# 2noise/ChatTTS

Hardware: AMD Instinct MI355X
Metric: audio seconds/sec (RTF), batch=64 per GPU (higher is better)
Workload: dtype f32x3

## Files before the change

### chattts_amd/_lib.py

```python
from __future__ import annotations

import ctypes as C
import os

import numpy as np

import torch

HERE = os.path.dirname(os.path.abspath(__file__))
LIB_PATH = os.environ.get("CTTS_LIB") or os.path.join(HERE, "csrc", "libchattts_amd.so")

F32, BF16 = 0, 1
P = C.c_void_p
PP = C.POINTER(C.c_void_p)


class GptWeights(C.Structure):
    _fields_ = [
        ("n_layers", C.c_int32), ("weight_dtype", C.c_int32), ("kv_dtype", C.c_int32), ("max_pos", C.c_int32),
        ("wqkv", PP), ("wo", PP), ("wgu", PP), ("wd", PP), ("ln1", PP), ("ln2", PP),
        ("norm", P), ("emb_code", P), ("heads", P), ("rope_cos", P), ("rope_sin", P),
        ("rms_eps", C.c_float),
        ("emb_text", P), ("head_text", P), ("n_text", C.c_int32),
        ("wqkv_pk", PP), ("wo_pk", PP), ("wgu_pk", PP), ("wd_pk", PP),
        ("heads_pk", P), ("head_text_pk", P),
        ("wo_hd", PP),
        ("wqkv_x3", PP), ("wo_x3", PP), ("wgu_x3", PP), ("wd_x3", PP),
    ]


class GenState(C.Structure):
    _fields_ = [
        ("B", C.c_int32), ("T", C.c_int32), ("max_new", C.c_int32),
        ("ids_buf", P), ("len", P), ("kv_start", P), ("finish", P), ("end_idx", P), ("hiddens", P),
        ("kcache", P), ("vcache", P), ("q", P), ("nq", C.c_int32),
        ("temperature", P), ("pow_table", P),
        ("top_p_thr", C.c_float), ("use_top_p", C.c_int32), ("top_k", C.c_int32), ("use_top_k", C.c_int32),
        ("min_new", C.c_int32), ("eos", C.c_int32), ("row_offset", C.c_int32),
        ("stop_at", P), ("workspace", P), ("workspace_bytes", C.c_size_t), ("row_map", P), ("n_active", P),
        ("cap", C.c_int32), ("hid_cap", C.c_int32), ("kv_batch", C.c_int32), ("q_batch", C.c_int32), ("prompt_len", P),
        ("infer_text", C.c_int32), ("teacher_ids", P), ("sampled_ids", P), ("order", P),
        ("rng_device", C.c_int32), ("rng_per_step", C.c_int32), ("rng_seed", P), ("rng_nonce", P),
# ... 106 lines not shown
    "ctts_dvae_encode_workspace_bytes": (SZ, [I32]),
    "ctts_dvae_decode_workspace_bytes": (SZ, [I32, I32]),
    "ctts_dvae_encode": (C.c_int, [P, P, I32, P, P, SZ, P]),
    "ctts_dvae_decode_codes": (C.c_int, [P, P, P, I32, I32, P, SZ, P]),
    "ctts_k_gemm": (C.c_int, [I32, P, P, P, I32, I32, I32, I32, I32, I32, I32, P, F, P, I32, P, P, I32, I32, I32, I32, I32, P]),
    "ctts_k_gemm_x3p": (C.c_int, [P, P, I32, I32, I32, I32, P, P, P, P, P, P]),
    "ctts_k_gemm_h1p": (C.c_int, [P, P, I32, I32, I32, I32, P, P, P, P, P, P]),
    "ctts_stream_create_cu_mask": (C.c_int, [I32, I32, I32, I32, P]),
    "ctts_stream_destroy": (C.c_int, [P]),
    "ctts_k_mlp_fused": (C.c_int, [P, P, P, I32, I32, P, P, P, P, I32, P]),
    "ctts_k_gemm_fast": (C.c_int, [P, I32, P, I32, I32, I32, P, F, I32, P, I32, P, I32, P, P]),
    "ctts_k_qkv_rope": (C.c_int, [P, P, I32, P, F, P, P, P, I32, P, P, I32, P, P, I32, P]),
    "ctts_k_gemm_dec": (C.c_int, [P, P, I32, I32, I32, P, P, F, I32, P, I32, P, I32, P, I32, P]),
    "ctts_k_gemm_dec32x": (C.c_int, [P, C.c_int64, P, C.c_int64, I32, I32, I32, P, P, I32, F, I32, P, I32, P, I32, P, C.c_int64, I32, P, I32, P, P, P]),
    "ctts_k_gemm_pre_x3": (C.c_int, [P, I32, P, P, I32, I32, I32, I32, I32, P, P, P, I32, P]),
    "ctts_k_dec32_last_variant": (C.c_char_p, []),
    "ctts_k_gemm_dec32": (C.c_int, [P, P, I32, I32, I32, P, P, I32, P, F, I32, P, I32, P, I32, P, I32, I32, I32, P]),
    "ctts_k_rows_prep": (C.c_int, [P, P, P, I32, P]),
    "ctts_k_rope_append": (C.c_int, [P, P, P, I32, I32, P, P, I32, P, P, I32, P]),
    "ctts_k_attention": (C.c_int, [P, P, P, I32, I32, P, I32, P, P, I32, P]),
    "ctts_k_attention_prefill": (C.c_int, [P, P, P, I32, P, I32, I32, P, I32, P]),
    "ctts_k_attention_dec": (C.c_int, [P, P, P, I32, P, P, P, I32, P, P, I32, P]),
    "ctts_k_attention_dec2": (C.c_int, [P, P, P, I32, I32, P, P, P, I32, I32, P]),
    "ctts_k_attention_cfg": (C.c_int, [I32, I32, I32]),
    "ctts_k_attention_heads_per_wg": (C.c_int, [I32]),
    "ctts_rccl_unique_id": (C.c_int, [P]),
    "ctts_rccl_comm_create": (C.c_int, [P, I32, P, I32]),
    "ctts_rccl_comm_destroy": (None, [P]),
    "ctts_broadcast_weights": (C.c_int, [P, P, I32, P, I32, P]),
    "ctts_k_attention_oproj": (C.c_int, [P, P, P, I32, P, P, P, I32, P, P, P, P, P, P]),
# ... 48 lines not shown
```

### chattts_amd/csrc/capi.hip

```cpp
#include <hip/hip_runtime.h>
#include <dlfcn.h>
#include <stdarg.h>
#include <stdio.h>
#include <stdlib.h>
#include <string.h>
#include <algorithm>
#include <map>
#include <vector>

#include "../../include/chattts_amd.h"
#include "kernels.hpp"

static thread_local char g_err[512] = "";
int ctts_fail(const char* fmt, ...) {
  va_list ap;
  va_start(ap, fmt);
  vsnprintf(g_err, sizeof(g_err), fmt, ap);
  va_end(ap);
  return -1;
}
#define fail ctts_fail
#define CK(expr)                                                                                   \
  do {                                                                                             \
    hipError_t _e = (expr);                                                                        \
// ... 11 lines not shown
  std::vector<const void*> wqkv_pk, wo_pk, wgu_pk, wd_pk;
  std::vector<const void*> wo_hd;
  std::vector<const void*> wqkv_x3, wo_x3, wgu_x3, wd_x3;
  bool dec_x3 = false;
  bool qkv_att = false;
  bool att_oproj = false;
  bool dec_packed = false;
  bool dec_packed32 = false;
  bool heads_packed = false;
  int pf_mask = 0;
  int temporal_layers = 0;
  bool pre32_packed = true;
  bool embed_fold = false;
  bool pre_compact = true;
  bool pre_x3 = true;
  bool fnorm_fuse = true;
  std::vector<const float*> ln1, ln2;
  hipGraph_t graph = nullptr;
  hipGraphExec_t exec = nullptr;
  hipGraph_t graph_multi = nullptr;
  hipGraphExec_t exec_multi = nullptr;
  struct RowsGraph { hipGraph_t graph = nullptr, gm = nullptr; hipGraphExec_t exec = nullptr, exec_multi = nullptr; };
  std::map<int, RowsGraph> rows_graphs;
  int multi_steps = 1;
  int prof_tag = -1;
  int prof_max = 0;
  bool skip_finished = true;
  int n_cu = 0;
  int prof_stride = 1;
  int prof_seen = 0;
// ... 92 lines not shown
    g->dec_x3 = true;
  }
  if (w->wo_hd && g->dec_packed) {
    g->wo_hd.assign(w->wo_hd, w->wo_hd + L);
    const char* e = getenv("CTTS_ATT_OPROJ");
    g->att_oproj = e && atoi(e) == 1;
  }
  { const char* e = getenv("CTTS_SKIP_FINISHED"); if (e && atoi(e) == 0) g->skip_finished = false; }
  { const char* e = getenv("CTTS_FNORM_FUSE"); if (e && atoi(e) == 0) g->fnorm_fuse = false; }
  { const char* e = getenv("CTTS_W_TEMPORAL_LAYERS"); if (e) g->temporal_layers = atoi(e); }
  { const char* e = getenv("CTTS_PF"); if (e) g->pf_mask = atoi(e); }
  { const char* e = getenv("CTTS_QKV_ATT"); g->qkv_att = e && atoi(e) == 1; }
  { const char* e = getenv("CTTS_PRE32_PACKED"); if (e && atoi(e) == 0) g->pre32_packed = false; }
  { const char* e = getenv("CTTS_PRE_X3"); if (e && atoi(e) == 0) g->pre_x3 = false; }
  { const char* e = getenv("CTTS_PRE_COMPACT"); if (e && atoi(e) == 0) g->pre_compact = false; }
  { const char* e = getenv("CTTS_EMBED_FOLD"); if (e) g->embed_fold = atoi(e) != 0; }
  {
    int dev = 0, cus = 0;
    const char* e = getenv("CTTS_ATT_SPLIT");
    if (e && atoi(e) == 1 && hipGetDevice(&dev) == hipSuccess &&
        hipDeviceGetAttribute(&cus, hipDeviceAttributeMultiprocessorCount, dev) == hipSuccess && cus > 0 && cus <= ATT_CUS_MAX)
      g->n_cu = cus;
  }
  *out = g;
  return 0;
}

extern "C" void ctts_gpt_graph_destroy(ctts_gpt* g) {
  if (!g) return;
  if (g->exec) { (void)hipGraphExecDestroy(g->exec); g->exec = nullptr; }
// ... 254 lines not shown
    d.epi = D32_EPI_QKV_ROPE; d.C = ws.qkv; d.ldc = 3 * HID; d.desc = ws.desc; d.cos_t = g->w.rope_cos; d.sin_t = g->w.rope_sin;
    d.kc = (float*)kc; d.vc = (float*)vc; d.cmax = cmax;
    CK(launch_gemm_pre32(d, ws.rstd, st));
    CK(launch_attention(ws.qkv, kc, vc, kt, cmax, ws.aop32, 3, rm, M, st));
    d.Ap = ws.aop32; d.Wp = (const float*)g->wo_pk[l]; d.N = HID; d.norm_w = nullptr; d.epi = EPI_RES; d.C = ws.x; d.ldc = HID;
    d.res = ws.x; d.ldr = HID; d.Cp = ws.xp32; d.kch_out = HID / 16;
    CK(launch_gemm_pre32(d, nullptr, st));
    CK(launch_rows_rstd32(ws.x, HID, M, g->w.rms_eps, ws.rstd, st));
    d.Ap = ws.xp32; d.Wp = (const float*)g->wgu_pk[l]; d.N = INTER; d.norm_w = g->ln2[l]; d.epi = EPI_SILU_MUL; d.C = nullptr;
    d.res = nullptr; d.Cp = ws.actp32; d.kch_out = INTER / 16;
    CK(launch_gemm_pre32(d, ws.rstd, st));
    d.Ap = ws.actp32; d.Wp = (const float*)g->wd_pk[l]; d.N = HID; d.K = INTER; d.norm_w = nullptr; d.epi = EPI_RES;
    d.C = ws.x; d.ldc = HID; d.res = ws.x; d.ldr = HID; d.Cp = ws.xp32; d.kch_out = HID / 16;
    CK(launch_gemm_pre32(d, nullptr, st));
  }
  for (int l = 0; !fast && !packed32 && !pre32 && !x3 && l < g->w.n_layers; ++l) {
    void* kc = (char*)s->kcache + kv_layer * l;
    void* vc = (char*)s->vcache + kv_layer * l;
    GemmArgs a;
    memset(&a, 0, sizeof(a));
    a.taps = 1;
    a.n_active = nact;
    a.A = ws.x; a.lda = HID; a.W = g->wqkv[l]; a.C = ws.qkv; a.ldc = 3 * HID; a.M = M; a.N = 3 * HID; a.K = HID; a.wt = wt;
    a.epi = EPI_STORE; a.norm_w = g->ln1[l]; a.eps = g->w.rms_eps;
    if (pre_x3) { CK(launch_rows_rstd32(ws.x, HID, M, g->w.rms_eps, ws.rstd, st)); CK(launch_gemm_pre_x3(a, ws.rstd, st)); }
    else { Prof p(g, 1, st, prof_ok); CK(launch_gemm_skinny(a, st)); }
    { Prof p(g, 2, st, prof_ok); CK(launch_rope_append(ws.qkv, kc, vc, kt, cmax, g->w.rope_cos, g->w.rope_sin, rm, M, st)); }
    { Prof p(g, 3, st, prof_ok); CK(launch_attention(ws.qkv, kc, vc, kt, cmax, ws.ao, 0, rm, M, st)); }
    a.A = ws.ao; a.lda = HID; a.W = g->wo[l]; a.C = ws.x; a.ldc = HID; a.N = HID; a.K = HID; a.epi = EPI_RES; a.norm_w = nullptr;
    a.res = ws.x; a.ldr = HID;
    if (pre_x3) CK(launch_gemm_pre_x3(a, nullptr, st));
// ... 837 lines not shown
}
extern "C" int ctts_k_final_norm(const float* x, int32_t q_per_b, const float* w, float eps, float* hfin, float* hiddens,
                                 int32_t max_new, const int32_t* len, int32_t T, int32_t B, void* stream) {
  CK(launch_final_norm(x, q_per_b, w, eps, hfin, hiddens, max_new, len, T, B, nullptr, nullptr, nullptr, (hipStream_t)stream));
  return 0;
}
extern "C" int ctts_k_gemm_pre_x3(const float* A, int32_t lda, const float* W, float* C, int32_t ldc, int32_t M, int32_t N, int32_t K, int32_t epi,
                                  const float* norm_w, const float* rstd, const float* res, int32_t ldr, void* stream) {
  GemmArgs a;
  memset(&a, 0, sizeof(a));
  a.taps = 1; a.A = A; a.lda = lda; a.W = W; a.C = C; a.ldc = ldc; a.M = M; a.N = N; a.K = K; a.wt = WT_F32; a.epi = epi;
  a.norm_w = norm_w; a.res = res; a.ldr = ldr;
  CK(launch_gemm_pre_x3(a, rstd, (hipStream_t)stream));
  return 0;
}
extern "C" int ctts_k_sample(const ctts_gen_state* s, const float* logits, void* stream) {
  if (!s || !logits) return fail("ctts_k_sample: bad arguments");
  CK(launch_sample(make_sample_args(s, logits), (hipStream_t)stream));
  return 0;
}
extern "C" int ctts_k_sample_text(const ctts_gen_state* s, const float* logits, int32_t n_text, void* stream) {
  if (!s || !logits || n_text <= 0 || n_text > NTEXT_MAX) return fail("ctts_k_sample_text: bad arguments");
  CK(launch_sample_text(make_sample_args(s, logits), n_text, (hipStream_t)stream));
  return 0;
}
extern "C" int ctts_k_device_guard_probe(void* stream, int32_t* before, int32_t* stream_dev, int32_t* inside, int32_t* switched) {
  if (!before || !stream_dev || !inside || !switched) return fail("ctts_k_device_guard_probe: null argument");
  int b = -1, in = -1;
  CK(hipGetDevice(&b));
  *stream_dev = -1;
// ... 252 lines not shown
```

### chattts_amd/csrc/gpt.hip

```cpp
#include <stdlib.h>

#include "common.hpp"
#include "kernels.hpp"
#include "decode_dev.hpp"

#ifndef CTTS_QF_DELAY
#define CTTS_QF_DELAY 8
#endif
#ifndef CTTS_QF_PRE
#define CTTS_QF_PRE 1
#endif
#define HID 768
#define NHEAD 12
#define HDIM 64
#define NVQ 4
#define NAUDIO 626

__device__ __forceinline__ void row_to_b_slot(const GptRowMap& rm, int m, int& b, int& slot) {
  if (rm.q_per_b == 1) { b = rm.row_map ? rm.row_map[m] : m; slot = rm.len[b] - 1; }
  else { b = m / rm.q_per_b; slot = rm.slot0 + m - b * rm.q_per_b; if (rm.row_map) b = rm.row_map[b]; }
}
__device__ __forceinline__ bool row_absent(const int32_t* n_active, int m) { return n_active != nullptr && m >= *n_active; }

__device__ __forceinline__ void emit_row(float4 s, int t, float* __restrict__ x_row, uint16_t* __restrict__ xb_row,
// ... 245 lines not shown
template <> __device__ __forceinline__ size_t pko_off<x3p_t>(int m, int c) { return pk_off(m, c, HID / 32); }
template <typename OT> __device__ __forceinline__ void store_out(OT* p, float v);
template <> __device__ __forceinline__ void store_out<x3p_t>(x3p_t* p, float v) { p->v = f32_to_bf16(v); }
template <typename OT> __device__ __forceinline__ void store_pko(OT* out, int m, int c, float v, size_t);
template <> __device__ __forceinline__ void store_pko<x3p_t>(x3p_t* out, int m, int c, float v, size_t plane) {
  uint16_t* p = reinterpret_cast<uint16_t*>(out) + pk_off(m, c, HID / 32);
  uint16_t h, l;
  x3_split(v, h, l);
  p[0] = h;
  p[plane] = l;
}
template <> __device__ __forceinline__ void store_out<float>(float* p, float v) { *p = v; }
template <> __device__ __forceinline__ void store_out<bf16_t>(bf16_t* p, float v) { *p = f32_to_bf16(v); }
template <> __device__ __forceinline__ void store_pko<float>(float* out, int m, int c, float v, size_t) { out[pko_off<float>(m, c)] = v; }
template <> __device__ __forceinline__ void store_pko<bf16_t>(bf16_t* out, int m, int c, float v, size_t) { out[pko_off<bf16_t>(m, c)] = f32_to_bf16(v); }

#ifndef CTTS_ATT_DPP
#define CTTS_ATT_DPP 1
#endif
template <int CTRL>
__device__ __forceinline__ float dpp_f(float v) {
  return __int_as_float(__builtin_amdgcn_update_dpp(__float_as_int(v), __float_as_int(v), CTRL, 0xf, 0xf, false));
}
template <int LPK>
__device__ __forceinline__ float group_sum(float d) {
#if CTTS_ATT_DPP
  d += dpp_f<0xB1>(d);
  d += dpp_f<0x4E>(d);
  d += dpp_f<0x141>(d);
  if (LPK == 16) d += dpp_f<0x140>(d);
// ... 314 lines not shown
    const u128* wo = reinterpret_cast<const u128*>(rm.wo_h) + (size_t)h * 8 * HID + tid;
#pragma unroll
    for (int jc = 0; jc < 3; ++jc)
#pragma unroll
      for (int g8 = 0; g8 < 8; ++g8) wv[jc][g8] = load16(wo + (size_t)g8 * HID + 256 * jc);
    __builtin_amdgcn_sched_barrier(0);
  }
  lrun = groups_sum<LPK>(lrun, lane);
#pragma unroll
  for (int e = 0; e < DPL; ++e) acc[e] = groups_sum<LPK>(acc[e], lane);
  if (NW == 1) {
    if (kg == 0) {
      const float inv = 1.0f / lrun;
      OT* op = PKO ? out + pko_off<OT>(m, h * HDIM + dl * DPL) : out + (size_t)m * HID + h * HDIM + dl * DPL;
#pragma unroll
      for (int e = 0; e < DPL; ++e) store_out<OT>(op + e, acc[e] * inv);
    }
    return;
  }
  if (kg == 0) {
    if (dl == 0) { sm_m[wave] = mrun; sm_l[wave] = lrun; }
#pragma unroll
    for (int e = 0; e < DPL; ++e) sm_acc[wave][dl * DPL + e] = acc[e];
  }
  __syncthreads();
  if (tid < HDIM) {
    float M = -INFINITY;
#pragma unroll
    for (int w = 0; w < NW; ++w) M = fmaxf(M, sm_m[w]);
    float L = 0.f, o = 0.f;
#pragma unroll
// ... 516 lines not shown
      CTTS_LAUNCH_SMEM((attention_k<bf16_t, 16, bf16_t, true>), grid, dim3(1024), att_lds, st, qkv, (const bf16_t*)kcache, (const bf16_t*)vcache, cmax, (bf16_t*)out, rm);
    else if (att_nbuf == 3)
      CTTS_LAUNCH_SMEM((attention_k<bf16_t, 4, bf16_t, true, false, false, 3>), grid, dim3(256), att_lds, st, qkv, (const bf16_t*)kcache, (const bf16_t*)vcache, cmax, (bf16_t*)out, rm);
    else
      CTTS_LAUNCH_SMEM((attention_k<bf16_t, 4, bf16_t, true>), grid, dim3(256), att_lds, st, qkv, (const bf16_t*)kcache, (const bf16_t*)vcache, cmax, (bf16_t*)out, rm);
    return hipGetLastError();
  }
  if (out_bf16 == 3 && !decode) {
    if (kv_wt == WT_BF16) return hipErrorInvalidValue;
    CTTS_LAUNCH((attention_k<float, 1, float, true>), grid, dim3(64), st, qkv, (const float*)kcache, (const float*)vcache, cmax, (float*)out, rm);
    return hipGetLastError();
  }
  if (out_bf16 == 4) {
    if (!decode || kv_wt == WT_BF16 || rm.x3_plane == 0) return hipErrorInvalidValue;
    CTTS_LAUNCH_SMEM((attention_k<float, 4, x3p_t, true>), grid, dim3(256), att_lds, st, qkv, (const float*)kcache, (const float*)vcache, cmax, (x3p_t*)out, rm);
    return hipGetLastError();
  }
  if (out_bf16 == 3) {
    if (!decode || kv_wt == WT_BF16) return hipErrorInvalidValue;
    if (att_nbuf == 3)
      CTTS_LAUNCH_SMEM((attention_k<float, 4, float, true, false, false, 3>), grid, dim3(256), att_lds, st, qkv, (const float*)kcache, (const float*)vcache, cmax, (float*)out, rm);
    else
      CTTS_LAUNCH_SMEM((attention_k<float, 4, float, true>), grid, dim3(256), att_lds, st, qkv, (const float*)kcache, (const float*)vcache, cmax, (float*)out, rm);
    return hipGetLastError();
  }
  if (decode && nw8 && kv_wt == WT_BF16 && out_bf16) {
    CTTS_LAUNCH((attention_k<bf16_t, 8, bf16_t>), grid, dim3(512), st, qkv, (const bf16_t*)kcache, (const bf16_t*)vcache, cmax, (bf16_t*)out, rm);
    return hipGetLastError();
  }
#define ATT(KT, NW, OT) CTTS_LAUNCH((attention_k<KT, NW, OT>), grid, dim3(64 * NW), st, qkv, (const KT*)kcache, (const KT*)vcache, cmax, (OT*)out, rm)
// ... 839 lines not shown
```

### chattts_amd/csrc/kernels.hpp

```cpp
#pragma once
#include <hip/hip_runtime.h>
#include <hip/hip_ext.h>
#include <stdint.h>

#include "common.hpp"

extern thread_local hipEvent_t ctts_prof_start, ctts_prof_stop;
#define CTTS_LAUNCH(kern, grid, block, st, ...)                                                                   \
  do {                                                                                                            \
    if (ctts_prof_start) {                                                                                        \
      hipExtLaunchKernelGGL(kern, grid, block, 0, st, ctts_prof_start, ctts_prof_stop, 0, __VA_ARGS__);           \
      ctts_prof_start = nullptr; ctts_prof_stop = nullptr;                                                        \
    } else {                                                                                                      \
      hipLaunchKernelGGL(kern, grid, block, 0, st, __VA_ARGS__);                                                  \
    }                                                                                                             \
  } while (0)

#define CTTS_LAUNCH_SMEM(kern, grid, block, smem, st, ...)                                                        \
  do {                                                                                                            \
    if (ctts_prof_start) {                                                                                        \
      hipExtLaunchKernelGGL(kern, grid, block, smem, st, ctts_prof_start, ctts_prof_stop, 0, __VA_ARGS__);        \
      ctts_prof_start = nullptr; ctts_prof_stop = nullptr;                                                        \
    } else {                                                                                                      \
      hipLaunchKernelGGL(kern, grid, block, smem, st, __VA_ARGS__);                                               \
// ... 30 lines not shown
  int wt;
  int epi;
  const float* norm_w;
  float eps;
  const float* res; int ldr;
  const float* bias;
  const float* gamma;
  const int32_t* n_active;
  int taps, cin, frames, pad, dil;
  long long* dbg;
  const int2* seg;
};

hipError_t launch_gemm_skinny(const GemmArgs& a, hipStream_t st);
hipError_t launch_gemm_pre_x3(const GemmArgs& a, const float* rstd, hipStream_t st);

enum FastEpi { FEPI_STORE32 = 0, FEPI_RES = 1, FEPI_SILU = 2, FEPI_QKV_ROPE = 3 };
#define SSQ_PARTS 48
struct FastGemmArgs {
  const uint16_t* A; int lda;
  const uint16_t* W;
  int M, N, K;
  const float* ssq_in;
  float eps;
  int epi;
  float* C32; int ldc;
  uint16_t* Cb; int ldcb;
  float* ssq_out;
  int q_per_b; const int32_t* len; const int32_t* kv_start;
  const int32_t* row_map;
// ... 338 lines not shown
```

### chattts_amd/csrc/prefill32x.hip

```cpp
#include <stdlib.h>

#include "common.hpp"
#include "kernels.hpp"

namespace {

constexpr int XBK = 32, XLD = XBK + 8;
constexpr int XNT = 256;

typedef float xf2 __attribute__((ext_vector_type(2)));
typedef _Float16 xb2 __attribute__((ext_vector_type(2)));

__device__ __forceinline__ void split2(const float a, const float b, uint32_t& hi, uint32_t& lo) {
  const xf2 v = {a > 65504.0f ? 65504.0f : (a < -65504.0f ? -65504.0f : a), b > 65504.0f ? 65504.0f : (b < -65504.0f ? -65504.0f : b)};
  const xb2 h = __builtin_convertvector(v, xb2);
  hi = __builtin_bit_cast(uint32_t, h);
  const xf2 hf = __builtin_convertvector(h, xf2);
  const xb2 l = __builtin_convertvector((v - hf) * X3_LO_SCALE, xb2);
  lo = __builtin_bit_cast(uint32_t, l);
}
__device__ __forceinline__ void split4(const float4 v, ushort4& hi, ushort4& lo) {
  uint32_t h0, l0, h1, l1;
  split2(v.x, v.y, h0, l0);
  split2(v.z, v.w, h1, l1);
// ... 143 lines not shown
  const dim3 grid(nx, small ? (a.M + 63) / 64 : (a.M + 127) / 128);
  switch (a.epi) {
    case EPI_SILU_MUL:
      if (small) CTTS_LAUNCH((gemm_pre_x3_k<EPI_SILU_MUL, 1>), grid, block, st, a, rstd); else CTTS_LAUNCH((gemm_pre_x3_k<EPI_SILU_MUL, 2>), grid, block, st, a, rstd);
      break;
    case EPI_RES:
      if (small) CTTS_LAUNCH((gemm_pre_x3_k<EPI_RES, 1>), grid, block, st, a, rstd); else CTTS_LAUNCH((gemm_pre_x3_k<EPI_RES, 2>), grid, block, st, a, rstd);
      break;
    case EPI_STORE:
      if (small) CTTS_LAUNCH((gemm_pre_x3_k<EPI_STORE, 1>), grid, block, st, a, rstd); else CTTS_LAUNCH((gemm_pre_x3_k<EPI_STORE, 2>), grid, block, st, a, rstd);
      break;
    default: return hipErrorInvalidValue;
  }
  return hipGetLastError();
}
```

### chattts_amd/engine.py

```python
from __future__ import annotations

import ctypes as C
import os
import logging
import math
from dataclasses import dataclass, field
from typing import Iterator, List, Optional, Sequence

import numpy as np
import torch

from . import _lib
from . import g711 as G711
from . import resample as RS
from . import timescale as TS
from ._sync import wait_event, wait_stream
from .config import DVAE, GPT, VOCOS
from .rng import ExpDraws, penalty_table
from .weights import fold_weight_norm, gpt_layer_count

log = logging.getLogger("chattts_amd")


@dataclass
# ... 136 lines not shown
    R, Cc = w.shape
    assert R % 16 == 0 and Cc % 32 == 0
    return w.reshape(R // 16, 16, Cc // 32, 4, 8).permute(0, 2, 3, 1, 4).contiguous()


X3_LO_SCALE = 2048.0


def split_f16(w: torch.Tensor):
    w = w.to(torch.float32).clamp(-65504.0, 65504.0)
    hi = w.to(torch.float16)
    lo = ((w - hi.to(torch.float32)) * X3_LO_SCALE).to(torch.float16)
    return hi, lo


def pack_frag_x3(w: torch.Tensor) -> torch.Tensor:
    hi, lo = split_f16(w)
    return torch.stack([pack_frag(hi), pack_frag(lo)], 0).contiguous()


def unpack_frag_x3(p: torch.Tensor, R: int, Cc: int) -> torch.Tensor:
    return unpack_frag(p[0].float(), R, Cc) + unpack_frag(p[1].float(), R, Cc) / X3_LO_SCALE


def pack_wo_heads(wo: torch.Tensor) -> torch.Tensor:
    assert tuple(wo.shape) == (GPT.hidden, GPT.hidden)
    return wo.view(GPT.hidden, GPT.n_heads, 8, 8).permute(1, 2, 0, 3).contiguous()


def pack_frag32(w: torch.Tensor) -> torch.Tensor:
# ... 30 lines not shown
            raise ValueError("dtype must be 'bf16' (perf), 'f32' (parity, exact float32) or 'f32x3' (parity, split-fp16 projections)")
        self.lib = _lib.lib()
        self.device = torch.device(device)
        if self.device.type != "cuda":
            raise _lib.EngineError("GptEngine needs a ROCm GPU device (there is no CPU path)")
        self.logger = logger
        self.dtype = dtype
        self.wdt = torch.bfloat16 if dtype == "bf16" else torch.float32
        self.code = _lib.BF16 if dtype == "bf16" else _lib.F32
        self.n_layers = gpt_layer_count(gpt_sd)
        self.max_pos = max_pos
        dev = self.device
        f = lambda t: t.to(torch.float32).contiguous().to(dev)
        wcast = lambda t: t.to(torch.float32).to(self.wdt).contiguous().to(dev)
        self.wqkv, self.wo, self.wgu, self.wd, self.ln1, self.ln2 = [], [], [], [], [], []
        fold = (lambda w, g: w.float() * g.float()[None, :]) if dtype == "bf16" else (lambda w, g: w)
        perm = rope_row_perm() if dtype == "bf16" else torch.arange(GPT.hidden)
        for i in range(self.n_layers):
            p = f"layers.{i}."
            ln1, ln2 = gpt_sd[p + "input_layernorm.weight"], gpt_sd[p + "post_attention_layernorm.weight"]
            self.wqkv.append(wcast(fold(torch.cat([gpt_sd[p + "self_attn.q_proj.weight"][perm], gpt_sd[p + "self_attn.k_proj.weight"][perm],
                                                   gpt_sd[p + "self_attn.v_proj.weight"]], 0), ln1)))
            self.wo.append(wcast(gpt_sd[p + "self_attn.o_proj.weight"]))
            self.wgu.append(wcast(fold(torch.cat([gpt_sd[p + "mlp.gate_proj.weight"], gpt_sd[p + "mlp.up_proj.weight"]], 0), ln2)))
            self.wd.append(wcast(gpt_sd[p + "mlp.down_proj.weight"]))
            self.ln1.append(f(gpt_sd[p + "input_layernorm.weight"]))
            self.ln2.append(f(gpt_sd[p + "post_attention_layernorm.weight"]))
        self.norm = f(gpt_sd["norm.weight"])
        self.emb_code = f(torch.stack([embed_sd[f"emb_code.{k}.weight"] for k in range(GPT.n_vq)], 0))
        self.emb_text = f(embed_sd["emb_text.weight"])
        self.heads = f(torch.cat([fold_weight_norm(embed_sd[f"head_code.{k}.parametrizations.weight.original0"].float(),
                                                   embed_sd[f"head_code.{k}.parametrizations.weight.original1"].float())
                                  for k in range(GPT.n_vq)], 0))
        self.head_text = f(fold_weight_norm(embed_sd["head_text.parametrizations.weight.original0"].float(),
                                            embed_sd["head_text.parametrizations.weight.original1"].float()))
        ng = float(self.norm.pow(2).mean().sqrt())
        self.logit_scale = {False: float(self.heads.pow(2).sum(1).mean().sqrt()) * ng, True: float(self.head_text.pow(2).sum(1).mean().sqrt()) * ng}
        cos, sin = rope_tables(max_pos, theta=rope_theta)
        self.rope_cos, self.rope_sin = cos.to(dev), sin.to(dev)
        self._arrs = [_lib.ptr_array(x) for x in (self.wqkv, self.wo, self.wgu, self.wd, self.ln1, self.ln2)]
# ... 3 lines not shown
        pk = pack_frag if dtype == "bf16" else pack_frag32
        self.packed, self._pk_arrs = None, None
        rp = rope_row_perm().to(dev)
        qk_perm = torch.cat([rp, GPT.hidden + rp, 2 * GPT.hidden + torch.arange(GPT.hidden, device=dev)])
        if use_packed and (dtype != "f32x3" or self.exact_fallback):
            self.packed = [[pk(t) for t in ws] for ws in (self.wqkv, self.wo, self.wgu, self.wd)]
            if dtype != "bf16":
                self.packed[0] = [pack_frag32(t[qk_perm]) for t in self.wqkv]
            self._pk_arrs = [_lib.ptr_array(x) for x in self.packed]
        self.x3, self._x3_arrs = None, None
        if use_packed and dtype == "f32x3":
            gain = lambda w_, g_: w_.float() * g_.float()[None, :]
            self.x3 = [[pack_frag_x3(gain(t[qk_perm], g_)) for t, g_ in zip(self.wqkv, self.ln1)], [pack_frag_x3(t) for t in self.wo],
                       [pack_frag_x3(gain(t, g_)) for t, g_ in zip(self.wgu, self.ln2)], [pack_frag_x3(t) for t in self.wd]]
            self._x3_arrs = [_lib.ptr_array(x) for x in self.x3]
        self.wo_hd = [pack_wo_heads(t) for t in self.wo] if (use_packed and dtype == "bf16" and os.environ.get("CTTS_ATT_OPROJ") == "1") else None
        self._wo_hd_arr = None if self.wo_hd is None else _lib.ptr_array(self.wo_hd)

        def pad16(t):
            r = (-t.shape[0]) % 16
            return t if r == 0 else torch.cat([t, torch.zeros((r, t.shape[1]), dtype=t.dtype, device=t.device)], 0)
        self.heads_pk = pack_frag32(pad16(self.heads)) if use_packed else None
        self.head_text_pk = pack_frag32(pad16(self.head_text)) if use_packed else None
        w = _lib.GptWeights()
        w.n_layers, w.weight_dtype, w.kv_dtype, w.max_pos = self.n_layers, self.code, self.code, max_pos
        w.wqkv, w.wo, w.wgu, w.wd, w.ln1, w.ln2 = [C.cast(a, _lib.PP) for a in self._arrs]
        w.norm, w.emb_code, w.heads = self.norm.data_ptr(), self.emb_code.data_ptr(), self.heads.data_ptr()
        w.rope_cos, w.rope_sin = self.rope_cos.data_ptr(), self.rope_sin.data_ptr()
        w.rms_eps = float(rms_eps)
        w.emb_text, w.head_text, w.n_text = self.emb_text.data_ptr(), self.head_text.data_ptr(), GPT.n_text
        if self._pk_arrs is not None:
            w.wqkv_pk, w.wo_pk, w.wgu_pk, w.wd_pk = [C.cast(a, _lib.PP) for a in self._pk_arrs]
        w.heads_pk, w.head_text_pk = _lib.ptr(self.heads_pk), _lib.ptr(self.head_text_pk)
        if self._wo_hd_arr is not None:
            w.wo_hd = C.cast(self._wo_hd_arr, _lib.PP)
        if self._x3_arrs is not None:
            w.wqkv_x3, w.wo_x3, w.wgu_x3, w.wd_x3 = [C.cast(a, _lib.PP) for a in self._x3_arrs]
        self._w = w
        h = C.c_void_p()
        _lib.check(self.lib.ctts_gpt_create(C.byref(h), C.byref(w)), "ctts_gpt_create")
        self.handle = h
        spec = codec_cu_spec() if os.environ.get("CTTS_GPT_COMPLEMENT") == "1" else None
        self.stream = cu_masked_stream(self.lib, dev, *spec, True) if spec else torch.cuda.Stream(device=dev)
        self._lane_res = [(self.handle, self.stream)]
        self._lane_res_alt = []
        self._lane_res_text = []
        self.default_lanes = 1
        self.rng = "host"
        self.last_stats = {}
        self._session = None
        self._session_alt = None
        self._session_text = None
# ... 1426 lines not shown
```

### include/chattts_amd.h

```cpp
#ifndef CHATTTS_AMD_H
#define CHATTTS_AMD_H

#include <stddef.h>
#include <stdint.h>

#ifdef __cplusplus
extern "C" {
#endif

#define CTTS_F32 0
#define CTTS_BF16 1

typedef struct ctts_gpt ctts_gpt;
typedef struct ctts_codec ctts_codec;

const char* ctts_last_error(void);
int ctts_version(void);

typedef struct {
  int32_t n_layers;
  int32_t weight_dtype;
  int32_t kv_dtype;
  int32_t max_pos;
  const void* const* wqkv;
// ... 10 lines not shown
  float rms_eps;
  const float* emb_text;
  const float* head_text;
  int32_t n_text;
  const void* const* wqkv_pk;
  const void* const* wo_pk;
  const void* const* wgu_pk;
  const void* const* wd_pk;
  const float* heads_pk;
  const float* head_text_pk;
  const void* const* wo_hd;
  const void* const* wqkv_x3;
  const void* const* wo_x3;
  const void* const* wgu_x3;
  const void* const* wd_x3;
} ctts_gpt_weights;

typedef struct {
  float temperature[4];
  float pow_table[17];
  int32_t use_penalty;
  float top_p_thr;
  int32_t use_top_p;
  int32_t top_k;
  int32_t use_top_k;
  int32_t min_new;
  int32_t reserved0;
  uint64_t rng_seed;
  int32_t rng_per_step;
  int32_t reserved1;
// ... 231 lines not shown
                    uint16_t* vcache, int32_t cmax, const float* cos_tab, const float* sin_tab, int32_t q_per_b, const int32_t* len,
                    const int32_t* kv_start, int32_t force_mb, void* stream);
int ctts_k_gemm_dec(const uint16_t* Ap, const uint16_t* Wp, int32_t M, int32_t N, int32_t K, const int32_t* n_active, const float* ssq_in,
                    float eps, int32_t epi, float* C32, int32_t ldc, uint16_t* Cp, int32_t kch_out, float* ssq_out, int32_t force_mb,
                    void* stream);
int ctts_k_gemm_dec32(const float* Ap, const float* Wp, int32_t M, int32_t N, int32_t K, const int32_t* n_active, const float* X, int32_t ldx,
                      const float* norm_w, float eps, int32_t epi, float* C, int32_t ldc, const float* res, int32_t ldr, float* Cp,
                      int32_t kch_out, int32_t force_mb, int32_t n_cols ,
                      void* stream);
int ctts_k_gemm_dec32x(const uint16_t* Ap, int64_t a_plane, const uint16_t* Wp, int64_t w_plane, int32_t M, int32_t N, int32_t K,
                       const int32_t* n_active, const float* X, int32_t ldx, float eps, int32_t epi, float* C, int32_t ldc, const float* res,
                       int32_t ldr, uint16_t* Cp, int64_t c_plane, int32_t kch_out, float* Cp32, int32_t force_mb, const float* ssq_in,
                       float* ssq_out, void* stream);
int ctts_k_gemm_pre_x3(const float* A, int32_t lda, const float* W, float* C, int32_t ldc, int32_t M, int32_t N, int32_t K, int32_t epi,
                       const float* norm_w, const float* rstd, const float* res, int32_t ldr, void* stream);
const char* ctts_k_dec32_last_variant(void);
int ctts_k_rows_prep(const float* x32, uint16_t* xb, float* ssq, int32_t M, void* stream);
int ctts_k_rope_append(float* qkv, void* kcache, void* vcache, int32_t kv_dtype, int32_t cmax, const float* cos_tab, const float* sin_tab,
                       int32_t q_per_b, const int32_t* len, const int32_t* kv_start, int32_t M, void* stream);
int ctts_k_attention(const float* qkv, const void* kcache, const void* vcache, int32_t kv_dtype, int32_t cmax, float* out,
                     int32_t q_per_b, const int32_t* len, const int32_t* kv_start, int32_t M, void* stream);
int ctts_k_attention_prefill(const float* qkv, const uint16_t* kcache, const uint16_t* vcache, int32_t cmax, float* out, int32_t q_per_b,
                             int32_t slot0, const int32_t* kv_start, int32_t M, void* stream);
int ctts_k_attention_dec(const float* qkv, const uint16_t* kcache, const uint16_t* vcache, int32_t cmax, uint16_t* out_packed,
                         const int32_t* desc, const int32_t* n_active, int32_t M, float* part, int32_t* cnt, int32_t n_cu, void* stream);
int ctts_k_attention_dec2(const float* qkv, const void* kcache, const void* vcache, int32_t kv_dtype, int32_t cmax, void* out_packed,
                          const int32_t* desc, const int32_t* n_active, int32_t covers_all, int32_t M, void* stream);
int ctts_k_attention_cfg(int32_t persist, int32_t workgroups, int32_t ring);
int ctts_k_attention_heads_per_wg(int32_t hpw);
int ctts_k_attention_oproj(const float* qkv, const uint16_t* kcache, const uint16_t* vcache, int32_t cmax, const uint16_t* wo_hd,
// ... 19 lines not shown
```

Before: 1060.

## Run prefill with pre-split f16 hi/lo planes and a 3-pass MFMA GEMM

Adds a prefill path for the f32x3 mode. Each RMSNorm'd input row is split once into f16 hi/lo planes by a new rows kernel, and weights are pre-split into hi/lo planes at load time. A new LDS-ring GEMM kernel streams both planes by DMA and runs three f16 MFMAs per tile, with SiLU-mul and residual epilogues that write split planes directly. Attention writes its output as split planes too. This replaces the earlier f32 prefill GEMM path, which presumably split operands on the fly. In exchange it stores an extra copy of the weights in device memory.

```diff
diff --git a/chattts_amd/_lib.py b/chattts_amd/_lib.py
--- a/chattts_amd/_lib.py
+++ b/chattts_amd/_lib.py
@@ -26,6 +26,7 @@
         ("heads_pk", P), ("head_text_pk", P),
         ("wo_hd", PP),
         ("wqkv_x3", PP), ("wo_x3", PP), ("wgu_x3", PP), ("wd_x3", PP),
+        ("wqkv_x3r", PP), ("wo_x3r", PP), ("wgu_x3r", PP), ("wd_x3r", PP),
     ]
 
 
@@ -162,6 +163,9 @@
     "ctts_k_gemm_dec": (C.c_int, [P, P, I32, I32, I32, P, P, F, I32, P, I32, P, I32, P, I32, P]),
     "ctts_k_gemm_dec32x": (C.c_int, [P, C.c_int64, P, C.c_int64, I32, I32, I32, P, P, I32, F, I32, P, I32, P, I32, P, C.c_int64, I32, P, I32, P, P, P]),
     "ctts_k_gemm_pre_x3": (C.c_int, [P, I32, P, P, I32, I32, I32, I32, I32, P, P, P, I32, P]),
+    "ctts_k_gemm_pre_x3p": (C.c_int, [P, C.c_int64, I32, P, C.c_int64, I32, I32, I32, I32, P, P, I32, P, I32, P, C.c_int64, I32, P]),
+    "ctts_k_rows_rstd32": (C.c_int, [P, I32, I32, F, P, P]),
+    "ctts_k_rows_rstd32_split": (C.c_int, [P, I32, P, I32, I32, F, P, P, C.c_int64, I32, P]),
     "ctts_k_dec32_last_variant": (C.c_char_p, []),
     "ctts_k_gemm_dec32": (C.c_int, [P, P, I32, I32, I32, P, P, I32, P, F, I32, P, I32, P, I32, P, I32, I32, I32, P]),
     "ctts_k_rows_prep": (C.c_int, [P, P, P, I32, P]),
diff --git a/chattts_amd/csrc/capi.hip b/chattts_amd/csrc/capi.hip
--- a/chattts_amd/csrc/capi.hip
+++ b/chattts_amd/csrc/capi.hip
@@ -49,6 +49,8 @@
   bool embed_fold = false;
   bool pre_compact = true;
   bool pre_x3 = true;
+  std::vector<const void*> wqkv_x3r, wo_x3r, wgu_x3r, wd_x3r;
+  bool pre_planes = false;
   bool fnorm_fuse = true;
   std::vector<const float*> ln1, ln2;
   hipGraph_t graph = nullptr;
@@ -171,6 +173,14 @@
   { const char* e = getenv("CTTS_PRE32_PACKED"); if (e && atoi(e) == 0) g->pre32_packed = false; }
   { const char* e = getenv("CTTS_PRE_X3"); if (e && atoi(e) == 0) g->pre_x3 = false; }
   { const char* e = getenv("CTTS_PRE_COMPACT"); if (e && atoi(e) == 0) g->pre_compact = false; }
+  if (g->dec_x3 && w->wqkv_x3r && w->wo_x3r && w->wgu_x3r && w->wd_x3r) {
+    g->wqkv_x3r.assign(w->wqkv_x3r, w->wqkv_x3r + L);
+    g->wo_x3r.assign(w->wo_x3r, w->wo_x3r + L);
+    g->wgu_x3r.assign(w->wgu_x3r, w->wgu_x3r + L);
+    g->wd_x3r.assign(w->wd_x3r, w->wd_x3r + L);
+    const char* e = getenv("CTTS_PREX3_PLANES");
+    g->pre_planes = !(e && atoi(e) == 0);
+  }
   { const char* e = getenv("CTTS_EMBED_FOLD"); if (e) g->embed_fold = atoi(e) != 0; }
   {
     int dev = 0, cus = 0;
@@ -455,7 +465,36 @@
     d.C = ws.x; d.ldc = HID; d.res = ws.x; d.ldr = HID; d.Cp = ws.xp32; d.kch_out = HID / 16;
     CK(launch_gemm_pre32(d, nullptr, st));
   }
-  for (int l = 0; !fast && !packed32 && !pre32 && !x3 && l < g->w.n_layers; ++l) {
+  const bool pre_planes = pre_x3 && g->pre_planes;
+  for (int l = 0; pre_planes && l < g->w.n_layers; ++l) {
+    void* kc = (char*)s->kcache + kv_layer * l;
+    void* vc = (char*)s->vcache + kv_layer * l;
+    uint16_t* xs = reinterpret_cast<uint16_t*>(ws.xp32);
+    uint16_t* aos = reinterpret_cast<uint16_t*>(ws.ao);
+    uint16_t* acts = reinterpret_cast<uint16_t*>(ws.act);
+    const size_t pl_h = (size_t)M * HID, pl_i = (size_t)M * INTER;
+    PreX3pArgs a;
+    memset(&a, 0, sizeof(a));
+    a.M = M;
+    CK(launch_rows_rstd32_split(ws.x, HID, g->ln1[l], M, HID, g->w.rms_eps, ws.rstd, xs, pl_h, HID, st));
+    a.A = xs; a.a_plane = pl_h; a.lda = HID; a.W = (const uint16_t*)g->wqkv_x3r[l]; a.w_plane = (size_t)3 * HID * HID; a.N = 3 * HID; a.K = HID;
+    a.epi = EPI_STORE; a.rstd = ws.rstd; a.C = ws.qkv; a.ldc = 3 * HID;
+    CK(launch_gemm_pre_x3p(a, st));
+    CK(launch_rope_append(ws.qkv, kc, vc, kt, cmax, g->w.rope_cos, g->w.rope_sin, rm, M, st));
+    rm.x3_plane = pl_h;
+    CK(launch_attention(ws.qkv, kc, vc, kt, cmax, aos, 5, rm, M, st));
+    a.A = aos; a.W = (const uint16_t*)g->wo_x3r[l]; a.w_plane = (size_t)HID * HID; a.N = HID; a.epi = EPI_RES; a.rstd = nullptr;
+    a.C = ws.x; a.ldc = HID; a.res = ws.x; a.ldr = HID;
+    CK(launch_gemm_pre_x3p(a, st));
+    CK(launch_rows_rstd32_split(ws.x, HID, g->ln2[l], M, HID, g->w.rms_eps, ws.rstd, xs, pl_h, HID, st));
+    a.A = xs; a.W = (const uint16_t*)g->wgu_x3r[l]; a.w_plane = (size_t)2 * INTER * HID; a.N = INTER; a.epi = EPI_SILU_MUL; a.rstd = ws.rstd;
+    a.C = nullptr; a.res = nullptr; a.Cp = acts; a.c_plane = pl_i; a.ldcp = INTER;
+    CK(launch_gemm_pre_x3p(a, st));
+    a.A = acts; a.a_plane = pl_i; a.lda = INTER; a.W = (const uint16_t*)g->wd_x3r[l]; a.w_plane = (size_t)HID * INTER; a.N = HID; a.K = INTER;
+    a.epi = EPI_RES; a.rstd = nullptr; a.C = ws.x; a.ldc = HID; a.res = ws.x; a.ldr = HID; a.Cp = nullptr;
+    CK(launch_gemm_pre_x3p(a, st));
+  }
+  for (int l = 0; !fast && !packed32 && !pre32 && !x3 && !pre_planes && l < g->w.n_layers; ++l) {
     void* kc = (char*)s->kcache + kv_layer * l;
     void* vc = (char*)s->vcache + kv_layer * l;
     GemmArgs a;
@@ -1323,6 +1362,28 @@
   CK(launch_gemm_pre_x3(a, rstd, (hipStream_t)stream));
   return 0;
 }
+extern "C" int ctts_k_gemm_pre_x3p(const uint16_t* A, int64_t a_plane, int32_t lda, const uint16_t* W, int64_t w_plane, int32_t M, int32_t N, int32_t K,
+                                   int32_t epi, const float* rstd, float* C, int32_t ldc, const float* res, int32_t ldr, uint16_t* Cp, int64_t c_plane,
+                                   int32_t ldcp, void* stream) {
+  if (a_plane <= 0 || w_plane <= 0 || (epi == EPI_SILU_MUL && c_plane <= 0)) return fail("ctts_k_gemm_pre_x3p: bad plane distance");
+  PreX3pArgs a;
+  memset(&a, 0, sizeof(a));
+  a.A = A; a.a_plane = (size_t)a_plane; a.lda = lda; a.W = W; a.w_plane = (size_t)w_plane; a.M = M; a.N = N; a.K = K; a.epi = epi; a.rstd = rstd;
+  a.C = C; a.ldc = ldc; a.res = res; a.ldr = ldr; a.Cp = Cp; a.c_plane = (size_t)c_plane; a.ldcp = ldcp;
+  CK(launch_gemm_pre_x3p(a, (hipStream_t)stream));
+  return 0;
+}
+extern "C" int ctts_k_rows_rstd32(const float* X, int32_t ldx, int32_t M, float eps, float* rstd, void* stream) {
+  if (!X || !rstd || M <= 0 || ldx < 768 || (ldx & 3)) return fail("ctts_k_rows_rstd32: bad arguments");
+  CK(launch_rows_rstd32(X, ldx, M, eps, rstd, (hipStream_t)stream));
+  return 0;
+}
+extern "C" int ctts_k_rows_rstd32_split(const float* X, int32_t ldx, const float* gain, int32_t M, int32_t K, float eps, float* rstd, uint16_t* planes,
+                                        int64_t plane, int32_t ldp, void* stream) {
+  if (plane <= 0 || ldx < K || ldp < K) return fail("ctts_k_rows_rstd32_split: bad arguments");
+  CK(launch_rows_rstd32_split(X, ldx, gain, M, K, eps, rstd, planes, (size_t)plane, ldp, (hipStream_t)stream));
+  return 0;
+}
 extern "C" int ctts_k_sample(const ctts_gen_state* s, const float* logits, void* stream) {
   if (!s || !logits) return fail("ctts_k_sample: bad arguments");
   CK(launch_sample(make_sample_args(s, logits), (hipStream_t)stream));
diff --git a/chattts_amd/csrc/gpt.hip b/chattts_amd/csrc/gpt.hip
--- a/chattts_amd/csrc/gpt.hip
+++ b/chattts_amd/csrc/gpt.hip
@@ -283,6 +283,18 @@
 template <> __device__ __forceinline__ void store_out<bf16_t>(bf16_t* p, float v) { *p = f32_to_bf16(v); }
 template <> __device__ __forceinline__ void store_pko<float>(float* out, int m, int c, float v, size_t) { out[pko_off<float>(m, c)] = v; }
 template <> __device__ __forceinline__ void store_pko<bf16_t>(bf16_t* out, int m, int c, float v, size_t) { out[pko_off<bf16_t>(m, c)] = f32_to_bf16(v); }
+struct x3r_t { uint16_t v; };
+template <> __device__ __forceinline__ size_t pko_off<x3r_t>(int m, int c) { return (size_t)m * HID + c; }
+template <> __device__ __forceinline__ void store_out<x3r_t>(x3r_t* p, float v) { p->v = f32_to_bf16(v); }
+template <> __device__ __forceinline__ void store_pko<x3r_t>(x3r_t*, int, int, float, size_t) {}
+template <typename OT> __device__ __forceinline__ void store_row(OT* p, float v, size_t) { store_out<OT>(p, v); }
+template <> __device__ __forceinline__ void store_row<x3r_t>(x3r_t* p, float v, size_t plane) {
+  uint16_t* q = reinterpret_cast<uint16_t*>(p);
+  uint16_t h, l;
+  x3_split(v, h, l);
+  q[0] = h;
+  q[plane] = l;
+}
 
 #ifndef CTTS_ATT_DPP
 #define CTTS_ATT_DPP 1
@@ -627,7 +639,7 @@
       const float inv = 1.0f / lrun;
       OT* op = PKO ? out + pko_off<OT>(m, h * HDIM + dl * DPL) : out + (size_t)m * HID + h * HDIM + dl * DPL;
 #pragma unroll
-      for (int e = 0; e < DPL; ++e) store_out<OT>(op + e, acc[e] * inv);
+      for (int e = 0; e < DPL; ++e) store_row<OT>(op + e, acc[e] * inv, rm.x3_plane);
     }
     return;
   }
@@ -1174,6 +1186,11 @@
   if (out_bf16 == 4) {
     if (!decode || kv_wt == WT_BF16 || rm.x3_plane == 0) return hipErrorInvalidValue;
     CTTS_LAUNCH_SMEM((attention_k<float, 4, x3p_t, true>), grid, dim3(256), att_lds, st, qkv, (const float*)kcache, (const float*)vcache, cmax, (x3p_t*)out, rm);
+    return hipGetLastError();
+  }
+  if (out_bf16 == 5) {
+    if (decode || kv_wt == WT_BF16 || rm.x3_plane == 0) return hipErrorInvalidValue;
+    CTTS_LAUNCH((attention_k<float, 1, x3r_t>), grid, dim3(64), st, qkv, (const float*)kcache, (const float*)vcache, cmax, (x3r_t*)out, rm);
     return hipGetLastError();
   }
   if (out_bf16 == 3) {
diff --git a/chattts_amd/csrc/kernels.hpp b/chattts_amd/csrc/kernels.hpp
--- a/chattts_amd/csrc/kernels.hpp
+++ b/chattts_amd/csrc/kernels.hpp
@@ -68,6 +68,19 @@
 
 hipError_t launch_gemm_skinny(const GemmArgs& a, hipStream_t st);
 hipError_t launch_gemm_pre_x3(const GemmArgs& a, const float* rstd, hipStream_t st);
+struct PreX3pArgs {
+  const uint16_t* A; size_t a_plane; int lda;
+  const uint16_t* W; size_t w_plane;
+  int M, N, K;
+  int epi;
+  const float* rstd;
+  float* C; int ldc;
+  const float* res; int ldr;
+  uint16_t* Cp; size_t c_plane; int ldcp;
+};
+hipError_t launch_gemm_pre_x3p(const PreX3pArgs& a, hipStream_t st);
+hipError_t launch_rows_rstd32_split(const float* X, int ldx, const float* g, int M, int K, float eps, float* rstd, uint16_t* P, size_t plane,
+                                    int ldp, hipStream_t st);
 
 enum FastEpi { FEPI_STORE32 = 0, FEPI_RES = 1, FEPI_SILU = 2, FEPI_QKV_ROPE = 3 };
 #define SSQ_PARTS 48
diff --git a/chattts_amd/csrc/prefill32x.hip b/chattts_amd/csrc/prefill32x.hip
--- a/chattts_amd/csrc/prefill32x.hip
+++ b/chattts_amd/csrc/prefill32x.hip
@@ -181,3 +181,200 @@
   }
   return hipGetLastError();
 }
+
+namespace {
+
+constexpr int PBK = 64, PNT = 512;
+#pragma clang diagnostic push
+#pragma clang diagnostic ignored "-Winline-asm"
+__device__ __forceinline__ void px_dma16(const void* g, uint32_t lds) {
+  asm volatile("s_mov_b32 m0, %1\n\ts_nop 0\n\tglobal_load_lds_dwordx4 %0, off" ::"v"(g), "s"(lds) : "memory", "m0");
+}
+#pragma clang diagnostic pop
+
+template <int EPI, int MBLK>
+__global__ __launch_bounds__(PNT) void gemm_pre_x3p_k(PreX3pArgs a) {
+  constexpr bool SILU = EPI == EPI_SILU_MUL;
+  constexpr int BM = 64 * MBLK;
+  constexpr int BNO = SILU ? 64 : 128;
+  constexpr int ROWS = 2 * BM + 256;
+  constexpr int SLOT = ROWS * PBK;
+  constexpr int NSLOT = MBLK == 1 ? 3 : 2;
+  constexpr int PW = ROWS / 8 / 8;
+  static_assert(4 * MBLK * 16 * 64 * 4 <= SLOT * 2, "the hand-over fits a slot");
+  __shared__ __attribute__((aligned(1024))) uint16_t ring[NSLOT * SLOT];
+  __shared__ float rstd_s[BM];
+
+  const int tid = threadIdx.x, lane = tid & 63;
+  const int wave = __builtin_amdgcn_readfirstlane(tid >> 6);
+  const int wm = wave & 1, wb = wave >> 1;
+  const int M = a.M, N = a.N, K = a.K;
+  const int m0 = blockIdx.y * BM, n0 = blockIdx.x * BNO;
+
+  if (a.rstd != nullptr && tid < BM) rstd_s[tid] = a.rstd[min(m0 + tid, M - 1)];
+  __syncthreads();
+
+  const uint16_t* src[PW];
+#pragma unroll
+  for (int q = 0; q < PW; ++q) {
+    const int sr = (wave + 8 * q) * 8 + (lane >> 3);
+    const int ch = (lane & 7) ^ ((sr >> 1) & 7);
+    if (sr < 2 * BM) {
+      const int pl = sr / BM, r = sr % BM;
+      src[q] = a.A + (size_t)pl * a.a_plane + (size_t)min(m0 + r, M - 1) * a.lda + ch * 8;
+    } else {
+      const int t = sr - 2 * BM, pl = t >> 7, r = t & 127;
+      const int gr = SILU ? (r < 64 ? n0 + r : N + n0 + (r - 64)) : n0 + r;
+      src[q] = a.W + (size_t)pl * a.w_plane + (size_t)gr * K + ch * 8;
+    }
+  }
+  const uint32_t ring_lds = (uint32_t)(uintptr_t)(__attribute__((address_space(3))) void*)ring + wave * 1024;
+  auto issue = [&](int kb) {
+    const uint32_t l = ring_lds + (kb % NSLOT) * (SLOT * 2);
+#pragma unroll
+    for (int q = 0; q < PW; ++q) px_dma16(src[q] + (size_t)kb * PBK, l + q * 8192);
+  };
+
+  f32x16 acc[MBLK], accx[MBLK];
+#pragma unroll
+  for (int i = 0; i < MBLK; ++i)
+#pragma unroll
+    for (int r = 0; r < 16; ++r) { acc[i][r] = 0.f; accx[i][r] = 0.f; }
+
+  const int ri = lane & 31, sw = (ri >> 1) & 7, kh = lane >> 5;
+  const int nk = K / PBK;
+#pragma unroll
+  for (int q = 0; q < NSLOT - 1; ++q)
+    if (q < nk) issue(q);
+  for (int s = 0; s < nk; ++s) {
+    if (NSLOT == 3 && s + 1 < nk) asm volatile("s_waitcnt vmcnt(%0)" ::"n"(PW) : "memory");
+    else asm volatile("s_waitcnt vmcnt(0)" ::: "memory");
+    __builtin_amdgcn_s_barrier();
+    if (s + NSLOT - 1 < nk) issue(s + NSLOT - 1);
+    const uint16_t* sl = ring + (s % NSLOT) * SLOT;
+#pragma unroll
+    for (int kk = 0; kk < PBK / 16; ++kk) {
+      const int co = ((kk * 2 + kh) ^ sw) * 8;
+      const uint16_t* wr = sl + (2 * BM + wb * 32 + ri) * PBK + co;
+      const f16x8 wh = *reinterpret_cast<const f16x8*>(wr);
+      const f16x8 wl = *reinterpret_cast<const f16x8*>(wr + 128 * PBK);
+#pragma unroll
+      for (int i = 0; i < MBLK; ++i) {
+        const uint16_t* ar = sl + ((wm * MBLK + i) * 32 + ri) * PBK + co;
+        const f16x8 ah = *reinterpret_cast<const f16x8*>(ar);
+        const f16x8 al = *reinterpret_cast<const f16x8*>(ar + BM * PBK);
+        f32x16 x = accx[i];
+        x = __builtin_amdgcn_mfma_f32_32x32x16_f16(al, wh, x, 0, 0, 0);
+        x = __builtin_amdgcn_mfma_f32_32x32x16_f16(ah, wl, x, 0, 0, 0);
+        accx[i] = x;
+        acc[i] = __builtin_amdgcn_mfma_f32_32x32x16_f16(ah, wh, acc[i], 0, 0, 0);
+      }
+    }
+  }
+
+#pragma unroll
+  for (int i = 0; i < MBLK; ++i)
+#pragma unroll
+    for (int r = 0; r < 16; ++r) acc[i][r] += accx[i][r] * X3_LO_INV;
+  const int cl = lane & 31;
+  if (SILU) {
+    __syncthreads();
+    float* xch = reinterpret_cast<float*>(ring) + (size_t)((wm * 2 + (wb & 1)) * MBLK) * (16 * 64) + lane;
+    if (wb >= 2) {
+#pragma unroll
+      for (int i = 0; i < MBLK; ++i)
+#pragma unroll
+        for (int r = 0; r < 16; ++r) xch[(i * 16 + r) * 64] = acc[i][r];
+    }
+    __syncthreads();
+    if (wb >= 2) return;
+#pragma unroll
+    for (int i = 0; i < MBLK; ++i) {
+#pragma unroll
+      for (int r = 0; r < 16; ++r) {
+        const int lrow = (wm * MBLK + i) * 32 + (r & 3) + 8 * (r >> 2) + 4 * (lane >> 5);
+        const int row = m0 + lrow;
+        if (row >= M) continue;
+        const float rs = a.rstd != nullptr ? rstd_s[lrow] : 1.0f;
+        const float up = xch[(i * 16 + r) * 64];
+        const float v = silu_f(acc[i][r] * rs) * (up * rs);
+        uint16_t h, l;
+        x3_split(v, h, l);
+        uint16_t* cp = a.Cp + (size_t)row * a.ldcp + n0 + wb * 32 + cl;
+        cp[0] = h;
+        cp[a.c_plane] = l;
+      }
+    }
+  } else {
+    const int col = n0 + wb * 32 + cl;
+#pragma unroll
+    for (int i = 0; i < MBLK; ++i) {
+#pragma unroll
+      for (int r = 0; r < 16; ++r) {
+        const int lrow = (wm * MBLK + i) * 32 + (r & 3) + 8 * (r >> 2) + 4 * (lane >> 5);
+        const int row = m0 + lrow;
+        if (row >= M) continue;
+        const float rs = a.rstd != nullptr ? rstd_s[lrow] : 1.0f;
+        const float v = acc[i][r] * rs;
+        a.C[(size_t)row * a.ldc + col] = (EPI == EPI_RES) ? a.res[(size_t)row * a.ldr + col] + v : v;
+      }
+    }
+  }
+}
+
+__global__ __launch_bounds__(256) void rows_rstd32_split_k(const float* __restrict__ X, int ldx, const float* __restrict__ g, int M, int K, float eps,
+                                                           float* __restrict__ rstd, uint16_t* __restrict__ P, size_t plane, int ldp) {
+  const int row = blockIdx.x * 4 + (threadIdx.x >> 6), lane = threadIdx.x & 63;
+  if (row >= M) return;
+  const float* x = X + (size_t)row * ldx;
+  const float r = wave_row_rstd(x, K, eps, lane);
+  if (lane == 0) rstd[row] = r;
+  uint16_t* p = P + (size_t)row * ldp;
+  for (int k = lane * 4; k < K; k += 256) {
+#pragma clang fp contract(off)
+    const float4 v = *reinterpret_cast<const float4*>(x + k);
+    const float4 w = *reinterpret_cast<const float4*>(g + k);
+    ushort4 h, l;
+    x3_split(v.x * w.x, h.x, l.x);
+    x3_split(v.y * w.y, h.y, l.y);
+    x3_split(v.z * w.z, h.z, l.z);
+    x3_split(v.w * w.w, h.w, l.w);
+    *reinterpret_cast<ushort4*>(p + k) = h;
+    *reinterpret_cast<ushort4*>(p + plane + k) = l;
+  }
+}
+
+}
+
+hipError_t launch_rows_rstd32_split(const float* X, int ldx, const float* g, int M, int K, float eps, float* rstd, uint16_t* P, size_t plane,
+                                    int ldp, hipStream_t st) {
+  if (M <= 0 || K <= 0 || (K & 3) || (ldx & 3) || (ldp & 3) || (plane & 3) || !X || !g || !rstd || !P) return hipErrorInvalidValue;
+  CTTS_LAUNCH(rows_rstd32_split_k, dim3((M + 3) / 4), dim3(256), st, X, ldx, g, M, K, eps, rstd, P, plane, ldp);
+  return hipGetLastError();
+}
+
+hipError_t launch_gemm_pre_x3p(const PreX3pArgs& a, hipStream_t st) {
+  if (a.M <= 0 || a.N <= 0 || a.K <= 0 || (a.K % PBK) || (a.lda & 7) || (a.a_plane & 7) || (a.w_plane & 7) || !a.A || !a.W) return hipErrorInvalidValue;
+  if (((uintptr_t)a.A & 15) || ((uintptr_t)a.W & 15)) return hipErrorInvalidValue;
+  if (a.epi == EPI_SILU_MUL ? ((a.N % 64) != 0 || !a.Cp || (a.ldcp < a.N)) : ((a.N % 128) != 0 || !a.C || a.ldc < a.N)) return hipErrorInvalidValue;
+  if (a.epi == EPI_RES && !a.res) return hipErrorInvalidValue;
+  const dim3 block(PNT);
+  const int nx = a.epi == EPI_SILU_MUL ? a.N / 64 : a.N / 128;
+  static int force_small = -1;
+  if (force_small < 0) { const char* e = getenv("CTTS_PREX3_SMALL"); force_small = e ? atoi(e) : 0; }
+  const bool small = force_small == 1 || (force_small != 2 && (long)nx * ((a.M + 127) / 128) < 1024);
+  const dim3 grid(nx, small ? (a.M + 63) / 64 : (a.M + 127) / 128);
+  switch (a.epi) {
+    case EPI_SILU_MUL:
+      if (small) CTTS_LAUNCH((gemm_pre_x3p_k<EPI_SILU_MUL, 1>), grid, block, st, a); else CTTS_LAUNCH((gemm_pre_x3p_k<EPI_SILU_MUL, 2>), grid, block, st, a);
+      break;
+    case EPI_RES:
+      if (small) CTTS_LAUNCH((gemm_pre_x3p_k<EPI_RES, 1>), grid, block, st, a); else CTTS_LAUNCH((gemm_pre_x3p_k<EPI_RES, 2>), grid, block, st, a);
+      break;
+    case EPI_STORE:
+      if (small) CTTS_LAUNCH((gemm_pre_x3p_k<EPI_STORE, 1>), grid, block, st, a); else CTTS_LAUNCH((gemm_pre_x3p_k<EPI_STORE, 2>), grid, block, st, a);
+      break;
+    default: return hipErrorInvalidValue;
+  }
+  return hipGetLastError();
+}
diff --git a/chattts_amd/engine.py b/chattts_amd/engine.py
--- a/chattts_amd/engine.py
+++ b/chattts_amd/engine.py
@@ -174,6 +174,26 @@
     return hi, lo
 
 
+def split_rows_x3(w: torch.Tensor) -> torch.Tensor:
+    hi, lo = split_f16(w)
+    return torch.stack([hi, lo], 0).contiguous()
+
+
+def layer_matrices(gpt_sd: dict, i: int, dtype: str):
+    fold = (lambda w, g: w.float() * g.float()[None, :]) if dtype == "bf16" else (lambda w, g: w)
+    perm = rope_row_perm() if dtype == "bf16" else torch.arange(GPT.hidden)
+    p = f"layers.{i}."
+    ln1, ln2 = gpt_sd[p + "input_layernorm.weight"], gpt_sd[p + "post_attention_layernorm.weight"]
+    wqkv = fold(torch.cat([gpt_sd[p + "self_attn.q_proj.weight"][perm], gpt_sd[p + "self_attn.k_proj.weight"][perm],
+                           gpt_sd[p + "self_attn.v_proj.weight"]], 0), ln1)
+    wgu = fold(torch.cat([gpt_sd[p + "mlp.gate_proj.weight"], gpt_sd[p + "mlp.up_proj.weight"]], 0), ln2)
+    return wqkv, gpt_sd[p + "self_attn.o_proj.weight"], wgu, gpt_sd[p + "mlp.down_proj.weight"]
+
+
+def prompt_planes_x3(mats) -> list:
+    return [split_rows_x3(t) for t in mats]
+
+
 def pack_frag_x3(w: torch.Tensor) -> torch.Tensor:
     hi, lo = split_f16(w)
     return torch.stack([pack_frag(hi), pack_frag(lo)], 0).contiguous()
@@ -234,16 +254,13 @@
         f = lambda t: t.to(torch.float32).contiguous().to(dev)
         wcast = lambda t: t.to(torch.float32).to(self.wdt).contiguous().to(dev)
         self.wqkv, self.wo, self.wgu, self.wd, self.ln1, self.ln2 = [], [], [], [], [], []
-        fold = (lambda w, g: w.float() * g.float()[None, :]) if dtype == "bf16" else (lambda w, g: w)
-        perm = rope_row_perm() if dtype == "bf16" else torch.arange(GPT.hidden)
         for i in range(self.n_layers):
             p = f"layers.{i}."
-            ln1, ln2 = gpt_sd[p + "input_layernorm.weight"], gpt_sd[p + "post_attention_layernorm.weight"]
-            self.wqkv.append(wcast(fold(torch.cat([gpt_sd[p + "self_attn.q_proj.weight"][perm], gpt_sd[p + "self_attn.k_proj.weight"][perm],
-                                                   gpt_sd[p + "self_attn.v_proj.weight"]], 0), ln1)))
-            self.wo.append(wcast(gpt_sd[p + "self_attn.o_proj.weight"]))
-            self.wgu.append(wcast(fold(torch.cat([gpt_sd[p + "mlp.gate_proj.weight"], gpt_sd[p + "mlp.up_proj.weight"]], 0), ln2)))
-            self.wd.append(wcast(gpt_sd[p + "mlp.down_proj.weight"]))
+            wqkv, wo, wgu, wd = layer_matrices(gpt_sd, i, dtype)
+            self.wqkv.append(wcast(wqkv))
+            self.wo.append(wcast(wo))
+            self.wgu.append(wcast(wgu))
+            self.wd.append(wcast(wd))
             self.ln1.append(f(gpt_sd[p + "input_layernorm.weight"]))
             self.ln2.append(f(gpt_sd[p + "post_attention_layernorm.weight"]))
         self.norm = f(gpt_sd["norm.weight"])
@@ -277,6 +294,10 @@
             self.x3 = [[pack_frag_x3(gain(t[qk_perm], g_)) for t, g_ in zip(self.wqkv, self.ln1)], [pack_frag_x3(t) for t in self.wo],
                        [pack_frag_x3(gain(t, g_)) for t, g_ in zip(self.wgu, self.ln2)], [pack_frag_x3(t) for t in self.wd]]
             self._x3_arrs = [_lib.ptr_array(x) for x in self.x3]
+        self.x3r, self._x3r_arrs = None, None
+        if self.x3 is not None and os.environ.get("CTTS_PREX3_PLANES", "1") != "0":
+            self.x3r = [prompt_planes_x3(ws) for ws in (self.wqkv, self.wo, self.wgu, self.wd)]
+            self._x3r_arrs = [_lib.ptr_array(x) for x in self.x3r]
         self.wo_hd = [pack_wo_heads(t) for t in self.wo] if (use_packed and dtype == "bf16" and os.environ.get("CTTS_ATT_OPROJ") == "1") else None
         self._wo_hd_arr = None if self.wo_hd is None else _lib.ptr_array(self.wo_hd)
 
@@ -299,6 +320,8 @@
             w.wo_hd = C.cast(self._wo_hd_arr, _lib.PP)
         if self._x3_arrs is not None:
             w.wqkv_x3, w.wo_x3, w.wgu_x3, w.wd_x3 = [C.cast(a, _lib.PP) for a in self._x3_arrs]
+        if self._x3r_arrs is not None:
+            w.wqkv_x3r, w.wo_x3r, w.wgu_x3r, w.wd_x3r = [C.cast(a, _lib.PP) for a in self._x3r_arrs]
         self._w = w
         h = C.c_void_p()
         _lib.check(self.lib.ctts_gpt_create(C.byref(h), C.byref(w)), "ctts_gpt_create")
diff --git a/include/chattts_amd.h b/include/chattts_amd.h
--- a/include/chattts_amd.h
+++ b/include/chattts_amd.h
@@ -48,6 +48,10 @@
   const void* const* wo_x3;
   const void* const* wgu_x3;
   const void* const* wd_x3;
+  const void* const* wqkv_x3r;
+  const void* const* wo_x3r;
+  const void* const* wgu_x3r;
+  const void* const* wd_x3r;
 } ctts_gpt_weights;
 
 typedef struct {
@@ -309,6 +313,12 @@
                        float* ssq_out, void* stream);
 int ctts_k_gemm_pre_x3(const float* A, int32_t lda, const float* W, float* C, int32_t ldc, int32_t M, int32_t N, int32_t K, int32_t epi,
                        const float* norm_w, const float* rstd, const float* res, int32_t ldr, void* stream);
+int ctts_k_gemm_pre_x3p(const uint16_t* A, int64_t a_plane, int32_t lda, const uint16_t* W, int64_t w_plane, int32_t M, int32_t N, int32_t K,
+                        int32_t epi, const float* rstd, float* C, int32_t ldc, const float* res, int32_t ldr, uint16_t* Cp, int64_t c_plane,
+                        int32_t ldcp, void* stream);
+int ctts_k_rows_rstd32(const float* X, int32_t ldx, int32_t M, float eps, float* rstd, void* stream);
+int ctts_k_rows_rstd32_split(const float* X, int32_t ldx, const float* gain, int32_t M, int32_t K, float eps, float* rstd, uint16_t* planes,
+                             int64_t plane, int32_t ldp, void* stream);
 const char* ctts_k_dec32_last_variant(void);
 int ctts_k_rows_prep(const float* x32, uint16_t* xb, float* ssq, int32_t M, void* stream);
 int ctts_k_rope_append(float* qkv, void* kcache, void* vcache, int32_t kv_dtype, int32_t cmax, const float* cos_tab, const float* sin_tab,
```

Measured after the change: 1051. No clear change (-0.8%).
